# shanghong/Multiband-RF-pulse-Design

Hardware: AMD Instinct MI355X
Metric: FIR designs/sec, n=512 taps m=16384 arbitrary-phase SOCP (fir_ap_cvx form) (higher is better)
Workload: dtype f64

## Files before the change

### include/mbfir.h

```cpp
#ifndef MBFIR_H
#define MBFIR_H

#ifdef __cplusplus
extern "C" {
#endif

#define MBFIR_SOLVED 0
#define MBFIR_INFEASIBLE 1
#define MBFIR_NUMERICAL 2
#define MBFIR_EARLY_FAIL 3
#define MBFIR_E_ARG (-1)
#define MBFIR_E_HIP (-2)
#define MBFIR_E_NODEVICE (-3)

typedef struct mbfir_ctx mbfir_ctx;

typedef struct mbfir_opts {
    int grid_m;
    int max_iter;
    double feastol;
    double abstol;
    double reltol;
    int refine;
    int verbose;
// ... 22 lines not shown
    int chol_launches;
    int builds;
    int dd_iters;
    int dd_kmax;
    int collectives;
    int lanes;
    int dd_form;
    double ms_cap;
    double cap_flop;
    double collective_bytes;
    int correctors;
    int correctors_taken;
    int gv_passes;
    int gtv_passes;
    int pair_passes;
} mbfir_info;

typedef int (*mbfir_allreduce_fn)(void* buf, long count, int op, void* user);

int  mbfir_comm_unique_id(mbfir_ctx* ctx, char* id128);
int  mbfir_comm_init(mbfir_ctx* ctx, int nranks, int rank, const char* id128);
void mbfir_comm_destroy(mbfir_ctx* ctx);
int  mbfir_test_comm_allreduce(mbfir_ctx* ctx, double* v, long n, int op);

mbfir_ctx*  mbfir_create(int device_id);
void        mbfir_destroy(mbfir_ctx* ctx);
const char* mbfir_last_error(mbfir_ctx* ctx);
void        mbfir_default_opts(mbfir_opts* opts);
void        mbfir_set_allreduce(mbfir_ctx* ctx, mbfir_allreduce_fn fn, void* user);
const char* mbfir_version(void);
// ... 139 lines not shown
```

### multiband-rf-pulse-design_amd/__init__.py

```python
import ctypes as C
import os

import numpy as np

_HERE = os.path.dirname(os.path.abspath(__file__))
LIB_PATH = os.path.join(_HERE, "libmbfir.so")

SOLVED, INFEASIBLE, NUMERICAL, EARLY_FAIL = 0, 1, 2, 3
E_ARG, E_HIP, E_NODEVICE = -1, -2, -3


class MbfirError(RuntimeError):
    pass


class Opts(C.Structure):
    _fields_ = [("grid_m", C.c_int), ("max_iter", C.c_int), ("feastol", C.c_double),
                ("abstol", C.c_double), ("reltol", C.c_double), ("refine", C.c_int),
                ("verbose", C.c_int), ("shard_rank", C.c_int), ("shard_size", C.c_int),
                ("dense_trig", C.c_int), ("ddkkt", C.c_int), ("lanes", C.c_int)]


class Info(C.Structure):
    _fields_ = [("status", C.c_int), ("iters", C.c_int), ("n_unknowns", C.c_int), ("n_rows", C.c_int),
                ("n_freq", C.c_int), ("n_lp", C.c_int), ("n_q3", C.c_int), ("n_big", C.c_int),
                ("pcost", C.c_double), ("dcost", C.c_double), ("gap", C.c_double), ("relgap", C.c_double),
                ("pres", C.c_double), ("dres", C.c_double),
                ("ms_assemble", C.c_double), ("ms_solve", C.c_double), ("ms_post", C.c_double),
                ("ms_total", C.c_double), ("ms_gram", C.c_double), ("ms_chol", C.c_double),
                ("gram_flop", C.c_double), ("gram_launches", C.c_int), ("lattice", C.c_int),
                ("chol_flop", C.c_double), ("chol_launches", C.c_int), ("builds", C.c_int),
                ("dd_iters", C.c_int), ("dd_kmax", C.c_int), ("collectives", C.c_int), ("lanes", C.c_int),
                ("dd_form", C.c_int), ("ms_cap", C.c_double), ("cap_flop", C.c_double),
                ("collective_bytes", C.c_double), ("correctors", C.c_int), ("correctors_taken", C.c_int),
                ("gv_passes", C.c_int), ("gtv_passes", C.c_int), ("pair_passes", C.c_int)]

    def as_dict(self):
        return {k: getattr(self, k) for k, _ in self._fields_}


class Job(C.Structure):
    _fields_ = [("which", C.c_int), ("n", C.c_int), ("nband", C.c_int), ("rc", C.c_int),
                ("f", C.POINTER(C.c_double)), ("a", C.POINTER(C.c_double)), ("d", C.POINTER(C.c_double)),
                ("params", C.c_double * 4), ("h_re", C.POINTER(C.c_double)), ("h_im", C.POINTER(C.c_double)),
                ("info", Info), ("z", C.POINTER(C.c_double)), ("z_cap", C.c_int), ("err", C.c_char * 128)]


class RemezJob(C.Structure):
    _fields_ = [("numtaps", C.c_int), ("nband", C.c_int), ("type", C.c_int), ("edges", C.POINTER(C.c_double)),
                ("desired", C.POINTER(C.c_double)), ("weight", C.POINTER(C.c_double)), ("h", C.POINTER(C.c_double)),
# ... 1137 lines not shown
```

### multiband-rf-pulse-design_amd/csrc/api.cpp

```cpp
#include "../../include/mbfir.h"
#include "program.h"
#include "pulse.h"
#include "solver.h"
#include <chrono>
#include <cmath>
#include <cstdio>
#include <algorithm>
#include <cstdlib>
#include <cstring>
#include <functional>
#include <atomic>
#include <condition_variable>
#include <map>
#include <mutex>
#include <memory>
#include <system_error>
#include <thread>

using namespace mbfir;

struct mbfir_ctx {
    std::unique_ptr<Solver> solver;
    int device = 0;
    std::vector<double> last_x;
// ... 48 lines not shown
    std::memset(info, 0, sizeof(*info));
    info->status = rc; info->iters = si.iters; info->n_unknowns = P.N();
    info->n_rows = si.n_rows; info->n_freq = si.n_freq;
    info->n_lp = P.l; info->n_q3 = P.nq3; info->n_big = P.big;
    info->pcost = si.pcost; info->dcost = si.dcost; info->gap = si.gap; info->relgap = si.relgap;
    info->pres = si.pres; info->dres = si.dres;
    info->ms_assemble = (t_asm - t0) + si.ms_assemble; info->ms_solve = si.ms_solve;
    info->ms_post = t_end - t_solved; info->ms_total = t_end - t0;
    info->ms_gram = si.ms_gram; info->ms_chol = si.ms_chol; info->gram_flop = si.gram_flop;
    info->gram_launches = si.lattice ? 0 : si.h_builds * (P.quad ? 3 : 1);
    info->lattice = si.lattice;
    info->chol_launches = si.chol_launches; info->chol_flop = si.chol_flop; info->builds = si.h_builds;
    info->dd_iters = si.dd_iters; info->dd_kmax = si.dd_kmax; info->lanes = si.lanes; info->collectives = si.collectives;
    info->collective_bytes = si.collective_bytes;
    info->ms_cap = si.ms_cap; info->cap_flop = si.cap_flop; info->dd_form = si.dd_iters > 0 ? si.dd_form : -1;
    info->correctors = si.correctors; info->correctors_taken = si.correctors_taken; info->gv_passes = si.gv_passes; info->gtv_passes = si.gtv_passes; info->pair_passes = si.pair_passes;
}

void taps_from_solution(Solver& solver, const TrigProgram& P, const std::vector<double>& x, int lane, double* h_re, double* h_im) {
    const int n = P.n;
    switch (P.which) {
        case DES_AP:
            solver.specfact_last(n, h_re, h_im, lane);
            break;
        case DES_LINPROG: {
            const int nh = P.nhalf;
            for (int i = 0; i < n; ++i) { h_re[i] = 0; h_im[i] = 0; }
            if (P.real_filter) {
                if (P.odd_filter) for (int k = 0; k < nh; ++k) { h_re[nh - 1 + k] = x[k]; h_re[nh - 1 - k] = x[k]; }
                else for (int k = 0; k < nh; ++k) { h_re[nh + k] = x[k]; h_re[nh - 1 - k] = x[k]; }
            } else if (P.odd_filter) {
// ... 850 lines not shown
```

### multiband-rf-pulse-design_amd/csrc/chol.hip

```cpp
#include "dev_common.h"
#include <algorithm>
#include <mutex>
#include <cstdlib>
#include <type_traits>

namespace mbfir {

constexpr int CB = 64;
constexpr int CLD = 66;

#ifdef CHOL_EXP_NO_MFMA
#define CHOL_KSTEPS(n) 1
#else
#define CHOL_KSTEPS(n) (n)
#endif
template <bool TRANSB>
__device__ __forceinline__ void mma64(const double (*As)[CLD], const double (*Bs)[CLD], int kbeg, int kend,
                                      v4d acc[2][2]) {
#ifdef CHOL_EXP_NO_MFMA
    kend = kbeg + 4;
#endif
    const int lane = threadIdx.x & 63, wv = threadIdx.x >> 6;
    const int wi = wv >> 1, wj = wv & 1;
    for (int k0 = kbeg; k0 < kend; k0 += 4) {
// ... 1427 lines not shown
    static int lose_now[64];
    static bool lose_init = false;
    int dev = 0;
    hipGetDevice(&dev);
    std::lock_guard<std::mutex> lk(lose_mu);
    if (!lose_init) { for (int& v : lose_now) v = -1; lose_init = true; }
    if (dev >= 0 && dev < 64 && lose != lose_now[dev]) {
        const int limit = lose >= 0 ? (1 << 14) : CHOL_SPIN_LIMIT_DEFAULT;
        hipMemcpyToSymbolAsync(HIP_SYMBOL(g_chol_lose_step), &lose, sizeof(int), 0, hipMemcpyHostToDevice, st);
        hipMemcpyToSymbolAsync(HIP_SYMBOL(g_chol_spin_limit), &limit, sizeof(int), 0, hipMemcpyHostToDevice, st);
        hipStreamSynchronize(st);
        lose_now[dev] = lose;
    }
}

int chol_inv_launch(double* H, double* M, double* Mt, double* W1, int np, int* flag, hipStream_t st, int split, bool poison,
                    double* Lcopy, hipEvent_t e0, hipEvent_t e1, int nlanes, size_t lane_bytes, const int* mask) {
    int launches = 0;
    const int nblk = np / CB;
    CholStep a;
    a.H = H; a.M = M; a.np = np; a.nblk = nblk;
    a.d0 = W1; a.Dfac = W1 + np; a.dinvG = W1 + (long)(CB + 1) * np; a.flag = flag;
    a.pivtol = 1e-13;
    a.lane_bytes = lane_bytes; a.mask = mask; a.nlanes = nlanes;
    a.sync = reinterpret_cast<int*>(W1 + (long)(CB + 2) * np);
    a.cnt = a.sync;
    a.Mt = Mt;
    if (split < 0) split = (nlanes >= 3 || np >= 4096) ? 4 : 0;
    if ((long)dag_cnt_ints(nblk) * 4 > ((long)np * np - (long)np) * 8) split = split == 4 ? (nlanes >= 3 ? 1 : 0) : split;
    const int nsync = split == 4 ? dag_cnt_ints(nblk) : nblk + 1;
    hipLaunchKernelGGL(k_chol_init, dim3(cdiv(std::max(np, nsync), 256), nlanes), dim3(256), 0, st, H, np, W1, flag, a.sync, nsync, lane_bytes, mask,
                       poison ? W1 + np : (double*)nullptr);
    if (e0) hipEventRecord(e0, st);
    if (split == 4) {
        int ntasks = 0;
        for (int k = 0; k <= nblk; ++k) ntasks += dag_step_tasks(dag_step(nblk, k));
        a.k = 0; a.phase = 1; a.nP = a.nMS = a.nT = a.nR = 0;
        a.ntasks = ntasks;
        hipLaunchKernelGGL(k_chol_dag, dim3(nlanes, ntasks), dim3(256), 0, st, a);
        if (e1) hipEventRecord(e1, st);
        if (Lcopy) hipLaunchKernelGGL(k_extract_L, dim3(cdiv((long)np * np, 256)), dim3(256), 0, st, H, np, a.Dfac, a.dinvG, Lcopy);
        return 1;
    }
    for (int k = 0; k <= nblk; ++k) {
        const int nrem = nblk - k - 1;
        a.k = k;
        a.nMS = k >= 1 ? 4 * k : 0;
// ... 170 lines not shown
```

### multiband-rf-pulse-design_amd/csrc/dev_common.h

```cpp
#pragma once
#include <hip/hip_runtime.h>
#include <cstdio>
#include <stdexcept>
#include <string>
#include <vector>

namespace mbfir {

struct HipError : std::runtime_error {
    explicit HipError(const std::string& s) : std::runtime_error(s) {}
};

#define MBFIR_HIP(expr)                                                                        \
    do {                                                                                       \
        hipError_t e__ = (expr);                                                               \
        if (e__ != hipSuccess)                                                                 \
            throw mbfir::HipError(std::string(#expr) + ": " + hipGetErrorString(e__) + " at " + \
                                  __FILE__ + ":" + std::to_string(__LINE__));                  \
    } while (0)

typedef double v4d __attribute__((ext_vector_type(4)));

__device__ __forceinline__ double wave_sum(double v) {
#pragma unroll
// ... 70 lines not shown
};
GramPlan gram_plan(int Mf, int Nt, int nw, int nlaunch = 1);
void gram_launch(const GramPlan& gp, const double* A, const double* d, double* slab, double* T,
                 const int* tile_ij, hipStream_t st, hipEvent_t ev0 = nullptr, hipEvent_t ev1 = nullptr, size_t d_stride = 0);
struct GramChunk { int plo = 0, phi = 0, blocks = 0, pair_off = 0; };
void gram_chunk_tables(const GramPlan& gp, int nchunks, std::vector<int>& table, std::vector<GramChunk>& chunks);
void gram_chunk_launch(const GramPlan& gp, const GramChunk& ck, const double* A, const double* d, double* slab,
                       const int* tile_ij, const int* chunk_table, double* Tp, hipStream_t st);
void gram_unpack_launch(const GramPlan& gp, const double* Tp, const int* tile_ij, const int* chunk_table, double* T, hipStream_t st);
int gram_grid_blocks(const GramPlan& gp);
int gram_table_ints(const GramPlan& gp);
void gram_tiles_host(const GramPlan& gp, int* tile_ij);

int chol_inv_launch(double* H, double* M, double* Mt, double* W1, int np, int* flag, hipStream_t st, int split, bool poison,
                    double* Lcopy = nullptr, hipEvent_t e0 = nullptr, hipEvent_t e1 = nullptr, int nlanes = 1,
                    size_t lane_bytes = 0, const int* mask = nullptr);
void chol_set_lose_step(int lose, hipStream_t st);

__global__ void k_extract_L_pub(const double* __restrict__ H, int np, const double* __restrict__ Dfac,
                                const double* __restrict__ dinvG, double* __restrict__ Lout);

void trigemv_launch(const double* T, int np, int upper, const double* b, double* y, int nv, int ldv,
                    hipStream_t st, const double* b2 = nullptr, int nlanes = 1, size_t lane_bytes = 0, const int* mask = nullptr);

bool hsolve_fused_ok(int np, int nv);
size_t hsolve_part_doubles(int np);
constexpr int HS_PARTS = 32;
void hsolve_launch(const double* M, int np, const double* b, const double* b2, double* out, double* part, int nv, int ldv,
                   hipStream_t st, int nlanes = 1, size_t lane_bytes = 0, const int* mask = nullptr, bool fold = true);

void dd_syrk_launch(const double* U, int ldu, const double* X, const int* kcount, int np, double* Hh, double* Hl,
// ... 26 lines not shown
```

### multiband-rf-pulse-design_amd/csrc/solver.h

```cpp
#pragma once
#include "program.h"
#include <stdexcept>
#include <string>
#include <vector>

namespace mbfir {

struct ShapeError : std::runtime_error {
    explicit ShapeError(const std::string& s) : std::runtime_error(s) {}
};
struct ResourceError : std::runtime_error {
    explicit ResourceError(const std::string& s) : std::runtime_error(s) {}
};

enum { ST_OPTIMAL = 0, ST_PRIMAL_INFEASIBLE = 1, ST_DUAL_INFEASIBLE = 2, ST_MAXIT = 3, ST_NUMERICAL = 4,
       ST_OPTIMAL_INACCURATE = 5 };

struct SolveOpts {
    int max_iter = 200;
    double feastol = 1e-8, abstol = 1e-10, reltol = 1e-8;
    int refine = 2;
    int verbose = 0;
    int shard_rank = 0, shard_size = 1;
    bool dense_trig = false;
// ... 5 lines not shown
struct SolveInfo {
    int status = 0, iters = 0, n_unknowns = 0, n_rows = 0, n_freq = 0;
    double pcost = 0, dcost = 0, gap = 0, relgap = 0, pres = 0, dres = 0;
    double ms_assemble = 0, ms_solve = 0, ms_gram = 0, ms_chol = 0, gram_flop = 0;
    int h_builds = 0;
    int chol_launches = 0;
    double chol_flop = 0;
    int dd_iters = 0, dd_kmax = 0;
    double ms_cap = 0, cap_flop = 0;
    int dd_form = 0;
    int collectives = 0;
    double collective_bytes = 0;
    int lanes = 1;
    int lattice = 0;
    int correctors = 0, correctors_taken = 0;
    int pair_passes = 0;
    int gv_passes = 0, gtv_passes = 0;
};

class Solver {
public:
    explicit Solver(int device);
    ~Solver();
    Solver(const Solver&) = delete;
    Solver& operator=(const Solver&) = delete;
    int solve(const TrigProgram& P, const SolveOpts& o, std::vector<double>& xout, SolveInfo& info);
    void solve_lanes(const std::vector<const TrigProgram*>& Ps, const SolveOpts& o, std::vector<std::vector<double>>& xouts,
                     std::vector<SolveInfo>& infos);
    static std::vector<long> shape_key(const TrigProgram& P, const SolveOpts& o);
    static int max_lanes(const TrigProgram& P, const SolveOpts& o);
// ... 25 lines not shown
```

### multiband-rf-pulse-design_amd/csrc/solver.hip

```cpp
#include "dev_common.h"
#include <functional>
#include <mutex>
#include <thread>
#include "cone_dev.h"
#include "dd_dev.h"
#include "program.h"
#include "solver.h"
#include <algorithm>
#include <chrono>
#include <cmath>
#include <cstdlib>
#include <cstring>
#include <vector>

#include <dlfcn.h>
#include <rccl/rccl.h>

namespace mbfir {

struct RcclApi {
    ncclResult_t (*GetUniqueId)(ncclUniqueId*) = nullptr;
    ncclResult_t (*CommInitRank)(ncclComm_t*, int, ncclUniqueId, int) = nullptr;
    ncclResult_t (*CommDestroy)(ncclComm_t) = nullptr;
    ncclResult_t (*AllReduce)(const void*, void*, size_t, ncclDataType_t, ncclRedOp_t, ncclComm_t, hipStream_t) = nullptr;
// ... 292 lines not shown
        }
    }
#pragma unroll
    for (int v = 0; v < NVV; ++v) {
        sh[wq][v][2 * lane] = acc[v].x;
        sh[wq][v][2 * lane + 1] = acc[v].y;
    }
    __syncthreads();
    for (int e = tid; e < NVV * 128; e += 256) {
        int v = e >> 7, cc = e & 127;
        double t = sh[0][v][cc] + sh[1][v][cc] + sh[2][v][cc] + sh[3][v][cc];
        partial[((long)split * NVV + v) * ld + blockIdx.x * 128 + cc] = t;
    }
}

__global__ __launch_bounds__(1024) void k_fold_partials(const double* __restrict__ partial, int nsplit, int nvv, int ld,
                                                        int ldo, double* __restrict__ TT, size_t lane_bytes, const int* lane_mask,
                                                        const LaneDims* __restrict__ dims, int cgrp) {
    LANES_RAW(lane_bytes, lane_mask, partial, TT);
    if (dims) nsplit = cgrp > 0 ? (dims[blockIdx.z].nchunk + cgrp - 1) / cgrp : (dims[blockIdx.z].Mown - cgrp - 1) / -cgrp;
    __shared__ double sh[16][65];
    const int c = threadIdx.x, sg = threadIdx.y, j = blockIdx.x * 64 + c, v = blockIdx.y;
    double t = 0;
    if (j < ld) {
        const double* p = partial + (long)v * ld + j;
        const long ss = (long)nvv * ld;
        int s = sg;
        for (; s + 48 < nsplit; s += 64) {
            const double a0 = p[s * ss], a1 = p[(s + 16) * ss], a2 = p[(s + 32) * ss], a3 = p[(s + 48) * ss];
            t += (a0 + a1) + (a2 + a3);
        }
        for (; s < nsplit; s += 16) t += p[s * ss];
    }
    sh[sg][c] = t;
    __syncthreads();
    if (sg == 0 && j < ld) {
        double a = 0;
// ... 1567 lines not shown
                    for (int f = 0; f < P.Ne; ++f)
                        acc[3 * e + f] += P.ey[3 * r + e] * sym3(m, a, b) * P.ey[3 * (r0 + b) + f];
        }
    }
    for (int e = 0; e < P.Ne; ++e)
        for (int f = 0; f < P.Ne; ++f) {
            double t = block_sum(acc[3 * e + f], sh);
            if (threadIdx.x == 0) H[(base + e) * ld + base + f] += t;
        }
}
__global__ __launch_bounds__(256) void k_H_yy(DProg P, const double* __restrict__ dl, const double* __restrict__ w3,
                                              double* __restrict__ H, long ld, long base, const double* __restrict__ m3c) {
    LANES(P, dl, w3, H, m3c);
    h_yy_block(P, dl, w3, H, ld, base, m3c, true);
}
__global__ __launch_bounds__(256) void k_pack_tril(const double* __restrict__ H, int np, double* __restrict__ out, int unpack) {
    const int t = blockIdx.x;
    int ti = int((sqrt(8.0 * t + 1.0) - 1.0) * 0.5);
    while ((long)(ti + 1) * (ti + 2) / 2 <= t) ++ti;
    while ((long)ti * (ti + 1) / 2 > t) --ti;
    const int tj = t - ti * (ti + 1) / 2;
    double* Hw = const_cast<double*>(H);
    for (int e = threadIdx.x; e < 64 * 32; e += 256) {
        const int r = e >> 5, c2 = 2 * (e & 31);
        double2* tile = reinterpret_cast<double2*>(out + (long)t * 4096 + r * 64 + c2);
        double2* mat = reinterpret_cast<double2*>(Hw + ((long)ti * 64 + r) * np + (long)tj * 64 + c2);
        if (unpack) *mat = *tile; else *tile = *mat;
    }
}
__global__ void k_zero3(double* __restrict__ a, long na, double* __restrict__ b, long nb, double* __restrict__ c, long nc, size_t lane_bytes, const int* lane_mask) {
// ... 107 lines not shown
    int test_cap_kp = 0;
    int ar_chunks = 0;
    int ar_overlap = 1;
    int cgrp = 4;
    int ddform = -1;
    bool dd_blockinv = true;
    bool hsolve = true;
    bool fuse = true;
    bool speculate = true;
    bool trace_host = false;
    int fold = -1;
    int chol_split = -1;
    bool poison = false;
    int test_lose_flag = -1;
    bool lanepair = true;
};
static SolveSwitches read_switches() {
    SolveSwitches w;
    auto flag = [](const char* name, bool& v) { if (const char* ev = std::getenv(name)) v = std::atoi(ev) != 0; };
    auto number = [](const char* name, int& v) { if (const char* ev = std::getenv(name)) v = std::atoi(ev); };
    flag("MBFIR_CORRECTOR", w.corrector); flag("MBFIR_CORR_BIG", w.corr_big); flag("MBFIR_DD_BLOCKINV", w.dd_blockinv);
    flag("MBFIR_HSOLVE", w.hsolve); flag("MBFIR_FUSE", w.fuse); flag("MBFIR_SPECULATE", w.speculate); flag("MBFIR_POISON", w.poison);
    flag("MBFIR_LANEPAIR", w.lanepair);
    number("MBFIR_TEST_CAP_KP", w.test_cap_kp); number("MBFIR_AR_OVERLAP", w.ar_overlap);
    number("MBFIR_CHOL_SPLIT", w.chol_split); number("MBFIR_TEST_LOSE_FLAG", w.test_lose_flag);
    if (const char* ev = std::getenv("MBFIR_CGRP")) w.cgrp = std::max(1, std::min(CGRP, std::atoi(ev)));
    if (const char* ev = std::getenv("MBFIR_AR_CHUNKS")) w.ar_chunks = std::max(1, std::atoi(ev));
    if (const char* ev = std::getenv("MBFIR_DDFORM")) w.ddform = std::strcmp(ev, "dd") != 0 ? 1 : 0;
    if (const char* ev = std::getenv("MBFIR_FOLD")) w.fold = std::atoi(ev) != 0;
    w.trace_host = std::getenv("MBFIR_TRACE_HOST") != nullptr;
    return w;
}

struct LatticeInfo {
    bool ok = false;
    double tmin = 0;
    int D1 = 0;
    std::vector<int> lat, lat_col, lat_qcol, ch_start, ch_count;
// ... 223 lines not shown
    return best;
}

struct Solver::Impl {
    int device = 0;
    hipStream_t st = nullptr;
    int shard_rank = 0, shard_size = 1;
    int (*ar_fn)(void*, long, int, void*) = nullptr;
    void* ar_user = nullptr;
    double* RB = nullptr;
    ncclComm_t comm = nullptr;
    int comm_size = 0, comm_rank = 0;
    long n_collectives = 0;
    double collective_bytes = 0;
    long n_pair = 0;
    long n_gv = 0, n_gtv = 0;
    void allreduce(double* buf, long count, int op, hipStream_t on = nullptr) {
        if (shard_size <= 1) return;
        if (!on) on = st;
        ++n_collectives;
        collective_bytes += 8.0 * double(count);
        if (comm) {
            ncclResult_t r = rccl().AllReduce(buf, buf, size_t(count), ncclDouble, op == 1 ? ncclMax : ncclSum, comm, on);
            if (r != ncclSuccess) throw HipError(std::string("ncclAllReduce: ") + (rccl().GetErrorString ? rccl().GetErrorString(r) : "failed"));
            return;
        }
        MBFIR_HIP(hipStreamSynchronize(on));
        if (!ar_fn || ar_fn(buf, count, op, ar_user) != 0) throw HipError("all-reduce hook failed");
    }
    hipEvent_t ev0 = nullptr, ev1 = nullptr;
// ... 164 lines not shown
        hipLaunchKernelGGL(k_rows_G<NV>, lane_grid(dim3(cdiv(P.R, 256)), nlanes), dim3(256), 0, st, P, UU, v, out);
    }
    template <int NV>
    void apply_G_winv2(const double* v, double* gout, const double* sub, double* wout) {
        if (P.trig && !P.big) {
            ++n_gv;
            trig_eval<NV>(v);
            hipLaunchKernelGGL(k_rows_winv2<NV>, lane_grid(dim3(cdiv(P.l + P.nq3, 256)), nlanes), dim3(256), 0, st, P, UU, v, dl, w3, sub, gout, wout);
            return;
        }
        apply_G<NV>(v, gout);
        winv2<NV>(gout, sub, wout, 0);
    }
    void moments_array(int nv, const double* pp, const double4* seeds, int na, int nb, double* out) {
        dim3 g(cdiv(na + nb, MPTS), cdiv(P.nchunk, P.cgrp)), b(256), gf(cdiv(P.nfold, 256));
        const bool pair = lane_pairs();
        if (pair) ++n_pair;
        switch (nv) {
#define MOM_CASE(NVX)                                                                                                          \
            case NVX:                                                                                                          \
                if (pp) hipLaunchKernelGGL((k_freq_fold<NVX, false>), lane_grid(gf, nlanes), b, 0, st, P, pp, PPf);            \
                if (pair) hipLaunchKernelGGL((k_trig_moments_pair<NVX, false>), lane_grid(g, cdiv(nlanes, 2)), b, 0, st, P, PPf, seeds, na, nb, partial, (const double*)nullptr, nlanes); \
                else hipLaunchKernelGGL((k_trig_moments<NVX>), lane_grid(g, nlanes), b, 0, st, P, PPf, seeds, na, nb, partial); \
                break;
            MOM_CASE(1) MOM_CASE(2) MOM_CASE(3) MOM_CASE(4) MOM_CASE(6)
#undef MOM_CASE
            default: throw HipError("moments: unsupported vector count");
        }
        hipLaunchKernelGGL(k_fold_partials, lane_grid(dim3(cdiv(P.LDM, 64), 2 * nv), nlanes), dim3(64, 16), 0, st, partial, cdiv(P.nchunk, P.cgrp), 2 * nv, P.LDM, P.LDM, out, lane_bytes, P.mask, P.dims, P.cgrp);
    }
    void atmulti_array(int nvv, const double* pp) {
        dim3 g(P.ld / 128, nsplit_at), b(64, 4);
        switch (nvv) {
            case 1: hipLaunchKernelGGL((k_atmulti<1, false>), lane_grid(g, nlanes), b, 0, st, P, A1, pp, partial); break;
            case 2: hipLaunchKernelGGL((k_atmulti<2, false>), lane_grid(g, nlanes), b, 0, st, P, A1, pp, partial); break;
            case 3: hipLaunchKernelGGL((k_atmulti<3, false>), lane_grid(g, nlanes), b, 0, st, P, A1, pp, partial); break;
            case 4: hipLaunchKernelGGL((k_atmulti<4, false>), lane_grid(g, nlanes), b, 0, st, P, A1, pp, partial); break;
            case 6: hipLaunchKernelGGL((k_atmulti<6, false>), lane_grid(g, nlanes), b, 0, st, P, A1, pp, partial); break;
            default: throw HipError("atmulti: unsupported vector count");
        }
    }
    template <int NV>
    void apply_GT(const double* val, double* out, int tail = 0, const double* rn_bx = nullptr, double* rn_r = nullptr, int rn_slot = 0) {
        ++n_gtv;
// ... 184 lines not shown
            hipEvent_t e;
            MBFIR_HIP(hipEventCreate(&e));
            evpool.push_back(e);
        }
        return evpool[evused++];
    }
    void build_H(int ddk = 0) {
        double* yy_sum = nullptr;
        const double* dlw = ddk > 0 ? D.dlc : dl;
        const double* m3c = ddk > 0 ? D.m3c : nullptr;
        const int* live_mask = P.mask;
        P.dd_lane = (dd_unit && ddk > 0) ? mask_row(ROW_DD) : nullptr;
        P.dl_plain = P.dd_lane ? dl : nullptr;
        const int nwv = P.quad ? 3 : 1, nvb = P.quad ? 2 * P.Ne : P.Ne;
        const bool one_pass = P.trig && P.Ne > 0 && P.tmin == 0.0 && nwv + nvb <= 4;
        if (!one_pass) hipLaunchKernelGGL(k_freq_blocks, lane_grid(dim3(cdiv(P.Mf, 256)), nlanes), dim3(256), 0, st, P, dlw, w3, Dw, BB, m3c);
        hipEvent_t g0 = timing ? next_event() : nullptr, g1 = timing ? next_event() : nullptr;
        if (P.trig) {
            if (g0) hipEventRecord(g0, st);
            const double* momb = MomB;
            if (one_pass) {
                hipLaunchKernelGGL(k_freq_blocks_fold, lane_grid(dim3(cdiv(P.nfold, 256)), nlanes), dim3(256), 0, st, P, dlw, w3, m3c, nwv + nvb, PPf);
                moments_array(nwv + nvb, nullptr, P.seed_h, P.D1, 2 * P.D1 - 1, Mom);
                momb = Mom + 2L * nwv * P.LDM;
            } else {
                moments_array(nwv, Dw, P.seed_h, P.D1, 2 * P.D1 - 1, Mom);
                if (P.Ne > 0) moments_array(nvb, BB, P.seed_tau, P.D1, 0, MomB);
            }
            if (lead_factor()) {
                yy_sum = nullptr;
                if (momb == MomB) {
                    allreduce(Mom, 2L * nwv * P.LDM, 0);
                    if (P.Ne > 0) allreduce(MomB, 2L * nvb * P.LDM, 0);
                } else {
                    long cnt = 2L * (nwv + nvb) * P.LDM;
                    if (P.Ne > 0 && cnt + 16 <= 18L * P.LDM) {
                        yy_sum = Mom + cnt;
                        hipMemsetAsync(yy_sum, 0, sizeof(double) * 9, st);
                        if (P.nyrows > 0) hipLaunchKernelGGL(k_H_yy, lane_grid(dim3(1), nlanes), dim3(256), 0, st, P, dlw, w3, yy_sum, 3L, 0L, m3c);
                        cnt += 9;
                    }
                    allreduce(Mom, cnt, 0);
                }
            }
            hipLaunchKernelGGL(k_assemble_H_lat, lane_grid(dim3((P.np / 64) * (P.np / 64 + 1) / 2, 16), nlanes), dim3(256), 0, st, P, Mom, momb, H, 1.0);
            if (g1) hipEventRecord(g1, st);
        } else {
        if (ar_overlap) {
            if (g0) hipEventRecord(g0, st);
            if (!st2) MBFIR_HIP(hipStreamCreateWithFlags(&st2, hipStreamNonBlocking));
            while (ovev.size() < 2 * gchunks.size()) { hipEvent_t e; MBFIR_HIP(hipEventCreateWithFlags(&e, hipEventDisableTiming)); ovev.push_back(e); }
            for (size_t c = 0; c < gchunks.size(); ++c) {
                const GramChunk& ck = gchunks[c];
                gram_chunk_launch(gps[0], ck, A1, Dw, slab, tile_ij, chunk_tab, Tp, st);
                if (shard_size > 1) {
                    MBFIR_HIP(hipEventRecord(ovev[2 * c], st));
                    MBFIR_HIP(hipStreamWaitEvent(st2, ovev[2 * c], 0));
                    allreduce(Tp + (size_t)ck.plo * 16384, (long)(ck.phi - ck.plo) * 16384, 0, st2);
                    MBFIR_HIP(hipEventRecord(ovev[2 * c + 1], st2));
// ... 2 lines not shown
            if (g1) hipEventRecord(g1, st);
        } else if (nlanes == 1) gram_launch(gps[0], A1, Dw, slab, T, tile_ij, st, g0, g1, P.Mpad);
        else {
        if (g0) hipEventRecord(g0, st);
        for (int b = 0; b < nlanes; ++b) {
            if (nlanes > 1 && !lane_live[b]) continue;
            const size_t off = (size_t)b * lane_bytes;
            auto at = [&](double* p) { return reinterpret_cast<double*>(reinterpret_cast<char*>(p) + off); };
            gram_launch(gps[b], at(A1), at(Dw), at(slab), at(T), reinterpret_cast<const int*>(reinterpret_cast<const char*>(tile_ij) + off), st, nullptr, nullptr, P.Mpad);
        }
        if (g1) hipEventRecord(g1, st);
        }
        if (P.Ne > 0) {
            int nvv = P.quad ? 2 * P.Ne : P.Ne;
            atmulti_array(nvv, BB);
            hipLaunchKernelGGL(k_fold_partials, lane_grid(dim3(cdiv(P.ld, 64), nvv), nlanes), dim3(64, 16), 0, st, partial, nsplit_at, nvv, P.ld, P.LDV, TT, lane_bytes, P.mask, P.dims, -AT_ROWS);
        }
        if (ar_overlap) {
            if (P.Ne > 0) {
                yy_sum = TT + (size_t)P.Ne * P.LDV;
                hipMemsetAsync(yy_sum, 0, sizeof(double) * 9, st);
                if (P.nyrows > 0) hipLaunchKernelGGL(k_H_yy, lane_grid(dim3(1), nlanes), dim3(256), 0, st, P, dlw, w3, yy_sum, 3L, 0L, m3c);
            }
            if (shard_size > 1) {
                MBFIR_HIP(hipStreamWaitEvent(st, ovev[2 * gchunks.size() - 1], 0));
                if (P.Ne > 0) allreduce(TT, (long)P.Ne * P.LDV + 9, 0);
            }
            gram_unpack_launch(gps[0], Tp, tile_ij, chunk_tab, T, st);
        }
        hipLaunchKernelGGL(k_assemble_H, lane_grid(dim3(cdiv(P.np, 256), P.np), nlanes), dim3(256), 0, st, P, T, TT, H, (ar_overlap || shard_rank == 0) ? 1.0 : 0.0);
        }
        const bool summed = shard_size > 1 && !lead_factor() && !ar_overlap;
        if (ar_overlap && P.Ne > 0) hipLaunchKernelGGL(k_H_yy_add, lane_grid(dim3(1), nlanes), dim3(16), 0, st, P, yy_sum, H);
        if (lead_factor() && P.Ne > 0) {
            const double* yy = yy_sum;
            if (!yy) {
                hipMemsetAsync(RB, 0, sizeof(double) * 9, st);
                if (P.nyrows > 0) hipLaunchKernelGGL(k_H_yy, lane_grid(dim3(1), nlanes), dim3(256), 0, st, P, dlw, w3, RB, 3L, 0L, m3c);
                allreduce(RB, 9, 0);
                yy = RB;
            }
            hipLaunchKernelGGL(k_H_yy_add, lane_grid(dim3(1), nlanes), dim3(16), 0, st, P, yy, H);
        }
        {
            const int yy_too = (!lead_factor() && !ar_overlap && P.Ne > 0 && P.nyrows > 0) ? 1 : 0;
            hipLaunchKernelGGL(k_H_identity, lane_grid(dim3(cdiv(P.Nt, 256) + yy_too), nlanes), dim3(256), 0, st, P, dlw, w3, H, m3c, yy_too, summed ? 1 : 0);
            if (P.big && (!summed || shard_rank == 0)) {
                memset_lanes(qv, sizeof(double) * 3 * P.LDV);
                if (ddk > 0) {
                    if (dd_unit) P.mask = mask_row(ROW_DD);
                    hipLaunchKernelGGL(k_big_q_dd, lane_grid(dim3(cdiv(P.big, 256)), nlanes), dim3(256), 0, st, P, D, qv, qv + P.LDV, qv + 2L * P.LDV);
                    hipLaunchKernelGGL(k_H_big_dd, lane_grid(dim3(cdiv(P.N, 256), P.N), nlanes), dim3(256), 0, st, P, D, qv, qv + P.LDV, qv + 2L * P.LDV, H);
                }
                if (ddk <= 0 || dd_unit) {
                    if (dd_unit && ddk > 0) P.mask = mask_row(ROW_PL);
                    hipLaunchKernelGGL(k_big_q, lane_grid(dim3(cdiv(P.big, 256)), nlanes), dim3(256), 0, st, P, wbb, qv, qv + P.LDV);
                    hipLaunchKernelGGL(k_H_big, lane_grid(dim3(cdiv(P.N, 256), P.N), nlanes), dim3(256), 0, st, P, qv, qv + P.LDV, Sc, H);
                }
                P.mask = live_mask;
            }
// ... 20 lines not shown
            P.mask = live_mask;
            hipEvent_t b0 = timing ? next_cap_event() : nullptr, b1 = timing ? next_cap_event() : nullptr;
            if (b0) hipEventRecord(b0, st);
            cap_build_launch(D.U, dd_unit ? kp : ddk, kp, P.np, M, D.sX, capYt, capZt, capS, capPart, st, nlanes, lb, mdd, dd_unit ? D.kcnt : nullptr);
            if (b1) hipEventRecord(b1, st);
            cap_flop_sum += 2.0 * (double(kp) * P.np * P.np + 0.5 * double(kp) * kp * P.np);
            chol_inv_launch(capS, capMs, nullptr, capW1, kp, capflag, st, sw.chol_split, sw.poison, nullptr, nullptr, c1, nlanes, lb, mdd);
            cap_flag_add_launch(flag, capflag, st, nlanes, lb, mdd);
        } else if (ddk > 0) {
            if (c0) hipEventRecord(c0, st);
            hipLaunchKernelGGL(k_dd_rows, lane_grid(dim3(ddk), nlanes), dim3(256), 0, st, P, D, P.np, ddk);
            dd_syrk_launch(D.U, P.np, D.sX, D.kcnt, P.np, H, M, st);
            dd_chol_launch(H, M, Mt, W1, ddri, ddri + P.np, ddd0, P.np, DD_PIVTOL, flag, st, ddinv);
            if (c1) hipEventRecord(c1, st);
        } else {
            chol_launch_count += chol_inv_launch(H, M, fused_hsolve ? nullptr : Mt, W1, P.np, flag, st, sw.chol_split, sw.poison, nullptr, c0, c1, nlanes, lane_bytes, P.mask);
        }
    }
    void prepare_lanes(const std::vector<const TrigProgram*>& Qs, const SolveOpts& o, std::vector<LaneHost>& LH) {
        shard_rank = o.shard_size > 1 ? o.shard_rank : 0;
        shard_size = o.shard_size > 1 ? o.shard_size : 1;
        if (shard_size > 1 && !ar_fn && !comm) throw HipError("row-sharded solve without a communicator or an all-reduce hook");
        if (comm && shard_size > 1 && (comm_size != shard_size || comm_rank != shard_rank))
            throw HipError("row-sharded solve: shard_rank / shard_size differ from the RCCL communicator's");
        n_collectives = 0; collective_bytes = 0;
        n_gv = 0; n_gtv = 0; n_pair = 0;
        if (shard_size > 1 && nlanes > 1) throw ShapeError("row-sharded solves run one design at a time");
        for (int b = 0; b < nlanes; ++b) {
            LaneHost& L = LH[b];
            const TrigProgram& Qfull = *Qs[b];
            if (shard_size > 1) { L.local = shard_program(Qfull, shard_rank, shard_size); L.Q = &L.local; }
            else L.Q = &Qfull;
            double nh = 0, nc = 0;
            for (double v : Qfull.h) nh += v * v;
            for (double v : Qfull.c) nc += v * v;
            L.nrm_h = std::max(1.0, std::sqrt(nh)); L.nrm_c = std::max(1.0, std::sqrt(nc));
            L.degree = double(Qfull.l + Qfull.nq3 + (Qfull.big ? 1 : 0));
            L.prep = lane_prep(*L.Q, o, sw);
            L.Lt = L.prep->Lt;
            L.nsweep = o.refine; L.nsweep_ctl = o.refine;
        }
// ... 440 lines not shown
        double ms_cap = 0;
        for (size_t i = 0; i + 1 < capev_used; i += 2) { float t = 0; hipEventElapsedTime(&t, capev[i], capev[i + 1]); ms_cap += t; }
        const int nw = P.quad ? 3 : 1;
        for (int b = 0; b < nlanes; ++b) {
            SolveInfo& info = infos[b];
            info = LH[b].info;
            info.status = LH[b].status;
            info.ms_assemble = t_assembled - t_begin;
            info.ms_solve = t_end - t_assembled;
            info.ms_gram = ms_gram; info.ms_chol = ms_chol; info.h_builds = builds;
            info.n_freq = LH[b].Q->Mf; info.n_rows = LH[b].Q->R; info.n_unknowns = LH[b].Q->N();
            info.lattice = P.trig;
            info.lanes = nlanes;
            info.collectives = int(n_collectives);
            info.collective_bytes = collective_bytes;
            info.gv_passes = int(n_gv); info.gtv_passes = int(n_gtv); info.pair_passes = int(n_pair);
            info.dd_iters = LH[b].dd_iters; info.dd_kmax = LH[b].dd_kmax;
            info.dd_form = cap_form ? 0 : 1; info.cap_flop = cap_flop_sum; info.ms_cap = ms_cap;
            info.chol_launches = int(chol_launch_count);
            info.chol_flop = 2.0 / 3.0 * double(P.np) * double(P.np) * double(P.np);
            info.gram_flop = P.trig ? double(3 * P.D1 - 1) * double(LH[b].Q->Mf) * (4.0 + 4.0 * nw)
                                    : double(nw) * double(P.Mf) * double(P.Nt) * double(P.Nt + 1);
        }
        nlanes_last = nlanes; taps_valid = false;
    }
};

Solver::Solver(int device) : impl(new Impl()) {
    impl->device = device;
    int ndev = 0;
    if (hipGetDeviceCount(&ndev) != hipSuccess || ndev <= 0) throw HipError("no HIP device available");
// ... 505 lines not shown
```

Baseline: 314.6.

## Fuse H tile assembly with identity, yy block and Cholesky init

Adds a tiled H-assembly kernel that builds each 64x64 lower-triangular tile of the lattice Gram matrix in shared memory. The same kernel also adds the identity/diagonal barrier contributions, the yy block and the Cholesky init (flag, sync counters, diagonal copy), so the separate k_H_identity and k_chol_init launches are skipped. Fold-partials is templated and defaults to a narrower 16-column block. The aim is fewer launches and fewer passes over H per iteration, at the cost of a more complex kernel with serial per-column sparse loops inside a single warp group and heavy shared-memory use.

```diff
diff --git a/include/mbfir.h b/include/mbfir.h
--- a/include/mbfir.h
+++ b/include/mbfir.h
@@ -60,6 +60,7 @@
     int gv_passes;
     int gtv_passes;
     int pair_passes;
+    int hbuild_fused;
 } mbfir_info;
 
 typedef int (*mbfir_allreduce_fn)(void* buf, long count, int op, void* user);
diff --git a/multiband-rf-pulse-design_amd/__init__.py b/multiband-rf-pulse-design_amd/__init__.py
--- a/multiband-rf-pulse-design_amd/__init__.py
+++ b/multiband-rf-pulse-design_amd/__init__.py
@@ -33,7 +33,7 @@
                 ("dd_iters", C.c_int), ("dd_kmax", C.c_int), ("collectives", C.c_int), ("lanes", C.c_int),
                 ("dd_form", C.c_int), ("ms_cap", C.c_double), ("cap_flop", C.c_double),
                 ("collective_bytes", C.c_double), ("correctors", C.c_int), ("correctors_taken", C.c_int),
-                ("gv_passes", C.c_int), ("gtv_passes", C.c_int), ("pair_passes", C.c_int)]
+                ("gv_passes", C.c_int), ("gtv_passes", C.c_int), ("pair_passes", C.c_int), ("hbuild_fused", C.c_int)]
 
     def as_dict(self):
         return {k: getattr(self, k) for k, _ in self._fields_}
diff --git a/multiband-rf-pulse-design_amd/csrc/api.cpp b/multiband-rf-pulse-design_amd/csrc/api.cpp
--- a/multiband-rf-pulse-design_amd/csrc/api.cpp
+++ b/multiband-rf-pulse-design_amd/csrc/api.cpp
@@ -86,7 +86,7 @@
     info->dd_iters = si.dd_iters; info->dd_kmax = si.dd_kmax; info->lanes = si.lanes; info->collectives = si.collectives;
     info->collective_bytes = si.collective_bytes;
     info->ms_cap = si.ms_cap; info->cap_flop = si.cap_flop; info->dd_form = si.dd_iters > 0 ? si.dd_form : -1;
-    info->correctors = si.correctors; info->correctors_taken = si.correctors_taken; info->gv_passes = si.gv_passes; info->gtv_passes = si.gtv_passes; info->pair_passes = si.pair_passes;
+    info->correctors = si.correctors; info->correctors_taken = si.correctors_taken; info->gv_passes = si.gv_passes; info->gtv_passes = si.gtv_passes; info->pair_passes = si.pair_passes; info->hbuild_fused = si.hbuild_fused;
 }
 
 void taps_from_solution(Solver& solver, const TrigProgram& P, const std::vector<double>& x, int lane, double* h_re, double* h_im) {
diff --git a/multiband-rf-pulse-design_amd/csrc/chol.hip b/multiband-rf-pulse-design_amd/csrc/chol.hip
--- a/multiband-rf-pulse-design_amd/csrc/chol.hip
+++ b/multiband-rf-pulse-design_amd/csrc/chol.hip
@@ -1465,8 +1465,22 @@
     }
 }
 
+static int chol_form(int np, int split, int nlanes) {
+    const int nblk = np / CB;
+    if (split < 0) split = (nlanes >= 3 || np >= 4096) ? 4 : 0;
+    if ((long)dag_cnt_ints(nblk) * 4 > ((long)np * np - (long)np) * 8) split = split == 4 ? (nlanes >= 3 ? 1 : 0) : split;
+    return split;
+}
+CholInit chol_init_layout(double* W1, int np, int* flag, int split, int nlanes) {
+    CholInit c;
+    c.d0 = W1; c.flag = flag;
+    c.sync = reinterpret_cast<int*>(W1 + (long)(CB + 2) * np);
+    c.nsync = chol_form(np, split, nlanes) == 4 ? dag_cnt_ints(np / CB) : np / CB + 1;
+    return c;
+}
+
 int chol_inv_launch(double* H, double* M, double* Mt, double* W1, int np, int* flag, hipStream_t st, int split, bool poison,
-                    double* Lcopy, hipEvent_t e0, hipEvent_t e1, int nlanes, size_t lane_bytes, const int* mask) {
+                    double* Lcopy, hipEvent_t e0, hipEvent_t e1, int nlanes, size_t lane_bytes, const int* mask, bool init_done) {
     int launches = 0;
     const int nblk = np / CB;
     CholStep a;
@@ -1477,11 +1491,11 @@
     a.sync = reinterpret_cast<int*>(W1 + (long)(CB + 2) * np);
     a.cnt = a.sync;
     a.Mt = Mt;
-    if (split < 0) split = (nlanes >= 3 || np >= 4096) ? 4 : 0;
-    if ((long)dag_cnt_ints(nblk) * 4 > ((long)np * np - (long)np) * 8) split = split == 4 ? (nlanes >= 3 ? 1 : 0) : split;
+    split = chol_form(np, split, nlanes);
     const int nsync = split == 4 ? dag_cnt_ints(nblk) : nblk + 1;
-    hipLaunchKernelGGL(k_chol_init, dim3(cdiv(std::max(np, nsync), 256), nlanes), dim3(256), 0, st, H, np, W1, flag, a.sync, nsync, lane_bytes, mask,
-                       poison ? W1 + np : (double*)nullptr);
+    if (!init_done || poison)
+        hipLaunchKernelGGL(k_chol_init, dim3(cdiv(std::max(np, nsync), 256), nlanes), dim3(256), 0, st, H, np, W1, flag, a.sync, nsync, lane_bytes, mask,
+                           poison ? W1 + np : (double*)nullptr);
     if (e0) hipEventRecord(e0, st);
     if (split == 4) {
         int ntasks = 0;
diff --git a/multiband-rf-pulse-design_amd/csrc/dev_common.h b/multiband-rf-pulse-design_amd/csrc/dev_common.h
--- a/multiband-rf-pulse-design_amd/csrc/dev_common.h
+++ b/multiband-rf-pulse-design_amd/csrc/dev_common.h
@@ -108,7 +108,9 @@
 
 int chol_inv_launch(double* H, double* M, double* Mt, double* W1, int np, int* flag, hipStream_t st, int split, bool poison,
                     double* Lcopy = nullptr, hipEvent_t e0 = nullptr, hipEvent_t e1 = nullptr, int nlanes = 1,
-                    size_t lane_bytes = 0, const int* mask = nullptr);
+                    size_t lane_bytes = 0, const int* mask = nullptr, bool init_done = false);
+struct CholInit { double* d0; int* flag; int* sync; int nsync; };
+CholInit chol_init_layout(double* W1, int np, int* flag, int split, int nlanes);
 void chol_set_lose_step(int lose, hipStream_t st);
 
 __global__ void k_extract_L_pub(const double* __restrict__ H, int np, const double* __restrict__ Dfac,
diff --git a/multiband-rf-pulse-design_amd/csrc/solver.h b/multiband-rf-pulse-design_amd/csrc/solver.h
--- a/multiband-rf-pulse-design_amd/csrc/solver.h
+++ b/multiband-rf-pulse-design_amd/csrc/solver.h
@@ -43,6 +43,7 @@
     int lanes = 1;
     int lattice = 0;
     int correctors = 0, correctors_taken = 0;
+    int hbuild_fused = 0;
     int pair_passes = 0;
     int gv_passes = 0, gtv_passes = 0;
 };
diff --git a/multiband-rf-pulse-design_amd/csrc/solver.hip b/multiband-rf-pulse-design_amd/csrc/solver.hip
--- a/multiband-rf-pulse-design_amd/csrc/solver.hip
+++ b/multiband-rf-pulse-design_amd/csrc/solver.hip
@@ -330,13 +330,14 @@
     }
 }
 
-__global__ __launch_bounds__(1024) void k_fold_partials(const double* __restrict__ partial, int nsplit, int nvv, int ld,
-                                                        int ldo, double* __restrict__ TT, size_t lane_bytes, const int* lane_mask,
-                                                        const LaneDims* __restrict__ dims, int cgrp) {
+template <int COLS>
+__global__ __launch_bounds__(COLS * 16) void k_fold_partials(const double* __restrict__ partial, int nsplit, int nvv, int ld,
+                                                             int ldo, double* __restrict__ TT, size_t lane_bytes, const int* lane_mask,
+                                                             const LaneDims* __restrict__ dims, int cgrp) {
     LANES_RAW(lane_bytes, lane_mask, partial, TT);
     if (dims) nsplit = cgrp > 0 ? (dims[blockIdx.z].nchunk + cgrp - 1) / cgrp : (dims[blockIdx.z].Mown - cgrp - 1) / -cgrp;
-    __shared__ double sh[16][65];
-    const int c = threadIdx.x, sg = threadIdx.y, j = blockIdx.x * 64 + c, v = blockIdx.y;
+    __shared__ double sh[16][COLS + 1];
+    const int c = threadIdx.x, sg = threadIdx.y, j = blockIdx.x * COLS + c, v = blockIdx.y;
     double t = 0;
     if (j < ld) {
         const double* p = partial + (long)v * ld + j;
@@ -1934,6 +1935,184 @@
     LANES(P, dl, w3, H, m3c);
     h_yy_block(P, dl, w3, H, ld, base, m3c, true);
 }
+constexpr int HT_IDENT = 1, HT_YY = 2, HT_INIT = 4;
+struct LatPair { double a, b; };
+__device__ __forceinline__ LatPair lat_T_load(const double* __restrict__ Mw, int LDM, int D1, int mj, int kj, int mk, int kk) {
+    const int d = mj - mk, ad = d < 0 ? -d : d, si = D1 + mj + mk;
+    const bool same = (kj == 0 && kk == 0) || (kj == 1 && kk == 1);
+    const double* A = same ? Mw : Mw + LDM;
+    return LatPair{A[ad], A[si]};
+}
+__device__ __forceinline__ double lat_T_value(LatPair m, int mj, int kj, double cj, int mk, int kk, double ck) {
+#pragma clang fp contract(off)
+    const bool same = (kj == 0 && kk == 0) || (kj == 1 && kk == 1);
+    const double sdv = mj - mk < 0 ? -m.a : m.a;
+    const double p = same ? m.a : m.b;
+    const double q = same ? (kj == 0 ? m.b : -m.b) : (kj == 0 ? -sdv : sdv);
+    return 0.5 * (p + q) * cj * ck;
+}
+__device__ __forceinline__ double lat_T_at(const double* __restrict__ Mw, int LDM, int D1, int mj, int kj, double cj, int mk, int kk, double ck) {
+    return lat_T_value(lat_T_load(Mw, LDM, D1, mj, kj, mk, kk), mj, kj, cj, mk, kk, ck);
+}
+template <bool ROWS>
+__device__ __forceinline__ void h_ident_tile(const DProg& P, const double* __restrict__ dl, const double* __restrict__ w3,
+                                             double (*tile)[64], int j, int j0, int k0) {
+#pragma clang fp contract(off)
+    const int own = ROWS ? j - j0 : j - k0;
+    auto add = [&](int k, double x, double y) {
+        const int o = ROWS ? k - k0 : k - j0;
+        if (o < 0 || o >= 64) return;
+        double& h = ROWS ? tile[own][o] : tile[o][own];
+        h = __builtin_fma(x, y, h);
+    };
+    for (int q = P.c_ptr[j]; q < P.c_ptr[j + 1]; ++q) {
+        const int r = P.c_rows[q];
+        const double al = P.alpha[r];
+        if (r < P.l) {
+            const double da = dl[r] * al;
+            if (ROWS) add(j, da, al);
+            for (int e = 0; e < P.Ne; ++e) add(P.Nt + e, da, P.ey[3 * r + e]);
+        } else if (r < P.l + 3 * P.nq3) {
+            const int c = (r - P.l) / 3, a = (r - P.l) - 3 * c, r0 = P.l + 3 * c;
+            double m[6];
+            load_m3(w3, nullptr, c, m);
+            for (int b = 0; b < 3; ++b) {
+                const double mm = sym3(m, a, b);
+                const int cb = P.col[r0 + b];
+                if (ROWS && cb >= 0) add(cb, al * P.alpha[r0 + b], mm);
+                const double am = al * mm;
+                for (int e = 0; e < P.Ne; ++e) add(P.Nt + e, am, P.ey[3 * (r0 + b) + e]);
+            }
+        }
+    }
+}
+__global__ __launch_bounds__(256) void k_assemble_H_tile(DProg P, const double* __restrict__ Mom, const double* __restrict__ MomB,
+                                                         const double* __restrict__ dl, const double* __restrict__ w3,
+                                                         double* __restrict__ H, CholInit I, int parts) {
+    LANES(P, Mom, MomB, dl, w3, H, I.d0, I.flag, I.sync);
+    __shared__ int s_lat[64], s_kind[64], s_plat[64], s_pkind[64];
+    __shared__ double s_scale[64], s_psign[64], s_pscale[64];
+    __shared__ double s_tile[64][64];
+    __shared__ double s_yy[9];
+    int ti = int((sqrt(8.0 * blockIdx.x + 1.0) - 1.0) * 0.5);
+    while ((ti + 1) * (ti + 2) / 2 <= int(blockIdx.x)) ++ti;
+    while (ti * (ti + 1) / 2 > int(blockIdx.x)) --ti;
+    const int tk = int(blockIdx.x) - ti * (ti + 1) / 2;
+    const int tid = threadIdx.x, c = tid & 63, g = tid >> 6, j0 = 64 * ti, k0 = 64 * tk, k = k0 + c;
+    if (parts & HT_INIT) {
+        if (blockIdx.x == 0 && tid == 0) I.flag[0] = 0;
+        for (int i = blockIdx.x * 256 + tid; i < I.nsync; i += gridDim.x * 256) I.sync[i] = 0;
+    }
+    if (tid < 64) {
+        const int j = j0 + tid;
+        int m = 0, kd = 0, pm = 0, pkd = 0;
+        double sc = 0, ps = 0, psc = 0;
+        if (j < P.Nt) {
+            m = P.lat[j]; kd = P.col_kind[j]; sc = P.col_scale[j];
+            if (P.quad) { const int pj = P.pcol[j]; ps = P.psign[j]; pm = P.lat[pj]; pkd = P.col_kind[pj]; psc = P.col_scale[pj]; }
+        }
+        s_lat[tid] = m; s_kind[tid] = kd; s_scale[tid] = sc; s_psign[tid] = ps; s_plat[tid] = pm; s_pkind[tid] = pkd; s_pscale[tid] = psc;
+    }
+    int mk = 0, kk = 0, pmk = 0, pkk = 0;
+    double sck = 0, psk = 0, psck = 0;
+    if (k < P.Nt) {
+        mk = P.lat[k]; kk = P.col_kind[k]; sck = P.col_scale[k];
+        if (P.quad) { const int pk = P.pcol[k]; psk = P.psign[k]; pmk = P.lat[pk]; pkk = P.col_kind[pk]; psck = P.col_scale[pk]; }
+    }
+    __syncthreads();
+    const long mw = 2L * P.LDM;
+    double v[16];
+    if (j0 + 64 <= P.Nt && k0 + 64 <= P.Nt) {
+#pragma clang fp contract(off)
+#pragma unroll
+        for (int i0 = 0; i0 < 16; i0 += 4) {
+            LatPair t0[4], t2[4], t1a[4], t1b[4];
+#pragma unroll
+            for (int u = 0; u < 4; ++u) {
+                const int r = g + 4 * (i0 + u);
+                t0[u] = lat_T_load(Mom, P.LDM, P.D1, s_lat[r], s_kind[r], mk, kk);
+                if (P.quad) {
+                    t2[u] = lat_T_load(Mom + 2 * mw, P.LDM, P.D1, s_plat[r], s_pkind[r], pmk, pkk);
+                    t1a[u] = lat_T_load(Mom + mw, P.LDM, P.D1, s_lat[r], s_kind[r], pmk, pkk);
+                    t1b[u] = lat_T_load(Mom + mw, P.LDM, P.D1, s_plat[r], s_pkind[r], mk, kk);
+                }
+            }
+#pragma unroll
+            for (int u = 0; u < 4; ++u) {
+                const int r = g + 4 * (i0 + u);
+                double x = lat_T_value(t0[u], s_lat[r], s_kind[r], s_scale[r], mk, kk, sck);
+                if (P.quad) {
+                    const double sj = s_psign[r];
+                    const double x2 = lat_T_value(t2[u], s_plat[r], s_pkind[r], s_pscale[r], pmk, pkk, psck);
+                    const double x1a = lat_T_value(t1a[u], s_lat[r], s_kind[r], s_scale[r], pmk, pkk, psck);
+                    const double x1b = lat_T_value(t1b[u], s_plat[r], s_pkind[r], s_pscale[r], mk, kk, sck);
+                    x = x + __builtin_fma(sj, x1b, __builtin_fma(sj * psk, x2, psk * x1a));
+                }
+                v[i0 + u] = x;
+            }
+        }
+    } else {
+#pragma clang fp contract(off)
+#pragma unroll 1
+        for (int i = 0; i < 16; ++i) {
+            const int r = g + 4 * i, j = j0 + r;
+            double x = 0;
+            if (j < P.Nt && k < P.Nt) {
+                x = lat_T_at(Mom, P.LDM, P.D1, s_lat[r], s_kind[r], s_scale[r], mk, kk, sck);
+                if (P.quad) {
+                    const double sj = s_psign[r];
+                    const double x2 = lat_T_at(Mom + 2 * mw, P.LDM, P.D1, s_plat[r], s_pkind[r], s_pscale[r], pmk, pkk, psck);
+                    const double x1a = lat_T_at(Mom + mw, P.LDM, P.D1, s_lat[r], s_kind[r], s_scale[r], pmk, pkk, psck);
+                    const double x1b = lat_T_at(Mom + mw, P.LDM, P.D1, s_plat[r], s_pkind[r], s_pscale[r], mk, kk, sck);
+                    x = x + __builtin_fma(sj, x1b, __builtin_fma(sj * psk, x2, psk * x1a));
+                }
+            } else if (j < P.N && k < P.N) {
+                const bool rowlow = j < k;
+                const int jj = rowlow ? j : k, e = (rowlow ? k : j) - P.Nt;
+                if (jj < P.Nt) {
+                    const int mjj = rowlow ? s_lat[r] : mk, kjj = rowlow ? s_kind[r] : kk;
+                    x = (rowlow ? s_scale[r] : sck) * MomB[((long)e * 2 + kjj) * P.LDM + mjj];
+                    if (P.quad) {
+                        const int pmjj = rowlow ? s_plat[r] : pmk, pkjj = rowlow ? s_pkind[r] : pkk;
+                        const double ps = (rowlow ? s_psign[r] : psk) * (rowlow ? s_pscale[r] : psck);
+                        x = __builtin_fma(ps, MomB[((long)(P.Ne + e) * 2 + pkjj) * P.LDM + pmjj], x);
+                    }
+                }
+            } else if (j == k) {
+                x = 1.0;
+            }
+            v[i] = x;
+        }
+    }
+    if (!(parts & HT_IDENT)) {
+#pragma unroll
+        for (int i = 0; i < 16; ++i) H[(long)(j0 + g + 4 * i) * P.np + k] = v[i];
+        return;
+    }
+#pragma unroll
+    for (int i = 0; i < 16; ++i) s_tile[g + 4 * i][c] = v[i];
+    const bool yrows_here = P.Nt < j0 + 64 && P.Nt + P.Ne > j0;
+    const bool yy_here = (parts & HT_YY) && yrows_here && P.Nt < k0 + 64 && P.Nt + P.Ne > k0;
+    if (yy_here && tid < 9) s_yy[tid] = -0.0;
+    __syncthreads();
+    if (g == 0) {
+        if (j0 + c < P.Nt) h_ident_tile<true>(P, dl, w3, s_tile, j0 + c, j0, k0);
+    } else if (g == 1 && yrows_here) {
+        if (k < P.Nt) h_ident_tile<false>(P, dl, w3, s_tile, k, j0, k0);
+    }
+    if (yy_here) {
+        h_yy_block(P, dl, w3, s_yy, 3L, 0L, nullptr, false);
+        __syncthreads();
+        if (tid < 9) {
+            const int e = tid / 3, f = tid - 3 * e, rr = P.Nt + e - j0, cc = P.Nt + f - k0;
+            if (e < P.Ne && f < P.Ne && rr >= 0 && rr < 64 && cc >= 0 && cc < 64) s_tile[rr][cc] += s_yy[tid];
+        }
+    }
+    __syncthreads();
+    if ((parts & HT_INIT) && ti == tk && tid < 64) I.d0[j0 + tid] = s_tile[tid][tid];
+#pragma unroll
+    for (int i = 0; i < 16; ++i) H[(long)(j0 + g + 4 * i) * P.np + k] = s_tile[g + 4 * i][c];
+}
 __global__ __launch_bounds__(256) void k_pack_tril(const double* __restrict__ H, int np, double* __restrict__ out, int unpack) {
     const int t = blockIdx.x;
     int ti = int((sqrt(8.0 * t + 1.0) - 1.0) * 0.5);
@@ -2071,6 +2250,8 @@
     bool poison = false;
     int test_lose_flag = -1;
     bool lanepair = true;
+    int hbuild = 1;
+    bool hbuild_pair = true;
 };
 static SolveSwitches read_switches() {
     SolveSwitches w;
@@ -2078,7 +2259,8 @@
     auto number = [](const char* name, int& v) { if (const char* ev = std::getenv(name)) v = std::atoi(ev); };
     flag("MBFIR_CORRECTOR", w.corrector); flag("MBFIR_CORR_BIG", w.corr_big); flag("MBFIR_DD_BLOCKINV", w.dd_blockinv);
     flag("MBFIR_HSOLVE", w.hsolve); flag("MBFIR_FUSE", w.fuse); flag("MBFIR_SPECULATE", w.speculate); flag("MBFIR_POISON", w.poison);
-    flag("MBFIR_LANEPAIR", w.lanepair);
+    flag("MBFIR_LANEPAIR", w.lanepair); flag("MBFIR_HBUILD_PAIR", w.hbuild_pair);
+    number("MBFIR_HBUILD", w.hbuild);
     number("MBFIR_TEST_CAP_KP", w.test_cap_kp); number("MBFIR_AR_OVERLAP", w.ar_overlap);
     number("MBFIR_CHOL_SPLIT", w.chol_split); number("MBFIR_TEST_LOSE_FLAG", w.test_lose_flag);
     if (const char* ev = std::getenv("MBFIR_CGRP")) w.cgrp = std::max(1, std::min(CGRP, std::atoi(ev)));
@@ -2332,6 +2514,7 @@
     long n_collectives = 0;
     double collective_bytes = 0;
     long n_pair = 0;
+    long n_hbuild = 0;
     long n_gv = 0, n_gtv = 0;
     void allreduce(double* buf, long count, int op, hipStream_t on = nullptr) {
         if (shard_size <= 1) return;
@@ -2526,7 +2709,7 @@
     }
     void moments_array(int nv, const double* pp, const double4* seeds, int na, int nb, double* out) {
         dim3 g(cdiv(na + nb, MPTS), cdiv(P.nchunk, P.cgrp)), b(256), gf(cdiv(P.nfold, 256));
-        const bool pair = lane_pairs();
+        const bool pair = lane_pairs() && sw.hbuild_pair;
         if (pair) ++n_pair;
         switch (nv) {
 #define MOM_CASE(NVX)                                                                                                          \
@@ -2539,7 +2722,11 @@
 #undef MOM_CASE
             default: throw HipError("moments: unsupported vector count");
         }
-        hipLaunchKernelGGL(k_fold_partials, lane_grid(dim3(cdiv(P.LDM, 64), 2 * nv), nlanes), dim3(64, 16), 0, st, partial, cdiv(P.nchunk, P.cgrp), 2 * nv, P.LDM, P.LDM, out, lane_bytes, P.mask, P.dims, P.cgrp);
+        fold_partials(cdiv(P.nchunk, P.cgrp), 2 * nv, P.LDM, P.LDM, out, P.cgrp);
+    }
+    void fold_partials(int nsplit, int nvv, int ld, int ldo, double* out, int cgrp) {
+        if (sw.hbuild) hipLaunchKernelGGL(k_fold_partials<16>, lane_grid(dim3(cdiv(ld, 16), nvv), nlanes), dim3(16, 16), 0, st, partial, nsplit, nvv, ld, ldo, out, lane_bytes, P.mask, P.dims, cgrp);
+        else hipLaunchKernelGGL(k_fold_partials<64>, lane_grid(dim3(cdiv(ld, 64), nvv), nlanes), dim3(64, 16), 0, st, partial, nsplit, nvv, ld, ldo, out, lane_bytes, P.mask, P.dims, cgrp);
     }
     void atmulti_array(int nvv, const double* pp) {
         dim3 g(P.ld / 128, nsplit_at), b(64, 4);
@@ -2754,6 +2941,9 @@
         P.dl_plain = P.dd_lane ? dl : nullptr;
         const int nwv = P.quad ? 3 : 1, nvb = P.quad ? 2 * P.Ne : P.Ne;
         const bool one_pass = P.trig && P.Ne > 0 && P.tmin == 0.0 && nwv + nvb <= 4;
+        const bool tile_path = sw.hbuild >= 1 && sw.hbuild <= 3 && P.trig && shard_size == 1 && !P.big && ddk <= 0 && !dd_unit;
+        const bool fuse_ident = tile_path && sw.hbuild != 2, fuse_init = fuse_ident && sw.hbuild == 1 && !sw.poison;
+        const int yy_too = (!lead_factor() && !ar_overlap && P.Ne > 0 && P.nyrows > 0) ? 1 : 0;
         if (!one_pass) hipLaunchKernelGGL(k_freq_blocks, lane_grid(dim3(cdiv(P.Mf, 256)), nlanes), dim3(256), 0, st, P, dlw, w3, Dw, BB, m3c);
         hipEvent_t g0 = timing ? next_event() : nullptr, g1 = timing ? next_event() : nullptr;
         if (P.trig) {
@@ -2783,6 +2973,12 @@
                     allreduce(Mom, cnt, 0);
                 }
             }
+            if (tile_path) {
+                const int parts = fuse_ident ? HT_IDENT | (yy_too ? HT_YY : 0) | (fuse_init ? HT_INIT : 0) : 0;
+                const CholInit ci = fuse_init ? chol_init_layout(W1, P.np, flag, sw.chol_split, nlanes) : CholInit{nullptr, nullptr, nullptr, 0};
+                hipLaunchKernelGGL(k_assemble_H_tile, lane_grid(dim3((P.np / 64) * (P.np / 64 + 1) / 2), nlanes), dim3(256), 0, st, P, Mom, momb, dlw, w3, H, ci, parts);
+                if (fuse_ident) ++n_hbuild;
+            } else
             hipLaunchKernelGGL(k_assemble_H_lat, lane_grid(dim3((P.np / 64) * (P.np / 64 + 1) / 2, 16), nlanes), dim3(256), 0, st, P, Mom, momb, H, 1.0);
             if (g1) hipEventRecord(g1, st);
         } else {
@@ -2815,7 +3011,7 @@
         if (P.Ne > 0) {
             int nvv = P.quad ? 2 * P.Ne : P.Ne;
             atmulti_array(nvv, BB);
-            hipLaunchKernelGGL(k_fold_partials, lane_grid(dim3(cdiv(P.ld, 64), nvv), nlanes), dim3(64, 16), 0, st, partial, nsplit_at, nvv, P.ld, P.LDV, TT, lane_bytes, P.mask, P.dims, -AT_ROWS);
+            fold_partials(nsplit_at, nvv, P.ld, P.LDV, TT, -AT_ROWS);
         }
         if (ar_overlap) {
             if (P.Ne > 0) {
@@ -2844,7 +3040,7 @@
             hipLaunchKernelGGL(k_H_yy_add, lane_grid(dim3(1), nlanes), dim3(16), 0, st, P, yy, H);
         }
         {
-            const int yy_too = (!lead_factor() && !ar_overlap && P.Ne > 0 && P.nyrows > 0) ? 1 : 0;
+            if (!fuse_ident)
             hipLaunchKernelGGL(k_H_identity, lane_grid(dim3(cdiv(P.Nt, 256) + yy_too), nlanes), dim3(256), 0, st, P, dlw, w3, H, m3c, yy_too, summed ? 1 : 0);
             if (P.big && (!summed || shard_rank == 0)) {
                 memset_lanes(qv, sizeof(double) * 3 * P.LDV);
@@ -2895,7 +3091,7 @@
             dd_chol_launch(H, M, Mt, W1, ddri, ddri + P.np, ddd0, P.np, DD_PIVTOL, flag, st, ddinv);
             if (c1) hipEventRecord(c1, st);
         } else {
-            chol_launch_count += chol_inv_launch(H, M, fused_hsolve ? nullptr : Mt, W1, P.np, flag, st, sw.chol_split, sw.poison, nullptr, c0, c1, nlanes, lane_bytes, P.mask);
+            chol_launch_count += chol_inv_launch(H, M, fused_hsolve ? nullptr : Mt, W1, P.np, flag, st, sw.chol_split, sw.poison, nullptr, c0, c1, nlanes, lane_bytes, P.mask, fuse_init);
         }
     }
     void prepare_lanes(const std::vector<const TrigProgram*>& Qs, const SolveOpts& o, std::vector<LaneHost>& LH) {
@@ -2905,7 +3101,7 @@
         if (comm && shard_size > 1 && (comm_size != shard_size || comm_rank != shard_rank))
             throw HipError("row-sharded solve: shard_rank / shard_size differ from the RCCL communicator's");
         n_collectives = 0; collective_bytes = 0;
-        n_gv = 0; n_gtv = 0; n_pair = 0;
+        n_gv = 0; n_gtv = 0; n_pair = 0; n_hbuild = 0;
         if (shard_size > 1 && nlanes > 1) throw ShapeError("row-sharded solves run one design at a time");
         for (int b = 0; b < nlanes; ++b) {
             LaneHost& L = LH[b];
@@ -3376,7 +3572,7 @@
             info.lanes = nlanes;
             info.collectives = int(n_collectives);
             info.collective_bytes = collective_bytes;
-            info.gv_passes = int(n_gv); info.gtv_passes = int(n_gtv); info.pair_passes = int(n_pair);
+            info.gv_passes = int(n_gv); info.gtv_passes = int(n_gtv); info.pair_passes = int(n_pair); info.hbuild_fused = int(n_hbuild);
             info.dd_iters = LH[b].dd_iters; info.dd_kmax = LH[b].dd_kmax;
             info.dd_form = cap_form ? 0 : 1; info.cap_flop = cap_flop_sum; info.ms_cap = ms_cap;
             info.chol_launches = int(chol_launch_count);
```

Result: no change. 316.5 (median of 6 runs) (+0.6%).
